# yixuan/ADMM

Measured on AMD Instinct MI355X. Metric: ADMM iterations/sec, Lasso tall n=100000 p=10000 (100-lambda warm-started path), higher is better.
Workload: dtype f32; 1 GPU; admm_lasso tall path (BASELINE configs[1]); n=100000, p=10000, nlambda=100, standardize=True, intercept=True, parallelism=single GPU, step=one cold-started warm-chained lambda path

## Files before the change

admm_amd/csrc/lasso_tall.hip:

```cpp
#include "prep.h"
#include "gemv_kernels.h"
#include "symv_kernels.h"
#include "solvers.h"
#include "sgl_host.h"
#include "box_host.h"
#include "comm.h"
#include "loop_driver.h"
#include "plan_host.h"
#include "peer_device.h"
#include "probe.h"

namespace admm {

struct TallCtl {
    double rho, lam, eps_primal, eps_dual, adj_a, adj_c, tau;
    double a_next, tau_next;
    int mode;
    int restart;
    int iter;
    int lam_idx;
    int done;
    int first;
    int total;
    int fin_idx;
    int fin_niter;
    int pad;
};

struct TallParams {
    int p, nwg, nseg, maxit, nlam, enet;
    long long part_stride;
    double eps_abs, eps_rel, alpha, sqrt_p;
    const double* lambdas;
    const float* XY;
    const float* a_part; const float* b_part;
    const float* dot0; const float* dot1; const float* axp0; const float* axp1;
    long long ldo; int nrb, p32; SymvSched sched;
    float* x; float* z0; float* z1; float* y0; float* y1; float* adj_z; float* adj_y; float* u; float* w;
    TallCtl* ctl;
    double* P;
    float* beta;
    int* niter;
    int* done_host;
#ifdef ADMM_HIP_PROBE
    long long* probe;
#endif
    double* trace;
    long long trace_cap;
    const float* refine_ab;
    long long refine_ld;
    float* state;
    long long state_cap;
    unsigned long long* verdict;
    unsigned long long* early;
    unsigned long long run_tag;
};

__host__ __device__ inline unsigned long long tall_verdict_word(unsigned long long run_tag, int total, bool discard) {
    return run_tag | ((unsigned long long)(unsigned)total << 1) | (discard ? 1ull : 0ull);
}
constexpr int kVerdictShift = 33;
constexpr int kVerdictWords = kSyVerdictReplicas * kSyVerdictStride;

constexpr int kTailThreads = 256;
constexpr int kGateCols = 3;
__host__ __device__ inline const double* tall_norm_rows(const double* P, int nwg, int par) { return P + (size_t)par * nwg * 8; }
__host__ __device__ inline size_t tall_norm_compact(int nwg, int par) { return (size_t)2 * nwg * 8 + (size_t)par * kGateCols * nwg; }
constexpr int kTailLanes = kSySumLanes;
constexpr int kTailElems = kTailThreads / kTailLanes;

__device__ __forceinline__ double tall_load_partial(const double* p, bool in_launch) {
    if (!in_launch) return *p;
    return __longlong_as_double((long long)__hip_atomic_load(reinterpret_cast<const unsigned long long*>(p), __ATOMIC_RELAXED, __HIP_MEMORY_SCOPE_AGENT));
}
__device__ __forceinline__ void tall_store_wt(float* p, float v) {
    __hip_atomic_store(reinterpret_cast<unsigned int*>(p), __float_as_uint(v), __ATOMIC_RELAXED, __HIP_MEMORY_SCOPE_AGENT);
}
__device__ __forceinline__ void tall_store_wt(double* p, double v) {
    __hip_atomic_store(reinterpret_cast<unsigned long long*>(p), (unsigned long long)__double_as_longlong(v), __ATOMIC_RELAXED, __HIP_MEMORY_SCOPE_AGENT);
}

enum { TALL_COLD = 0, TALL_CONVERGED = 1, TALL_ACCELERATE = 2, TALL_RESTART = 3 };
struct TallOutcome {
    int code;
    int fin;
    int done;
    double rp, rd, c;
    __device__ __forceinline__ bool discard() const { return code == TALL_CONVERGED || done != 0; }
    __device__ __forceinline__ int pick() const { return code == TALL_RESTART ? 1 : 0; }
};

template <int NK> struct TallNormReq { double v[2][NK]; };
template <int NK, bool IN_LAUNCH>
__device__ __forceinline__ TallNormReq<NK> tall_norms_request(const double* Pin, int nwg, int rs, int cs) {
    TallNormReq<NK> r;
#pragma unroll
    for (int j = 0; j < 2; ++j) {
        const int w = min((int)threadIdx.x + j * kTailThreads, nwg - 1);
#pragma unroll
        for (int k = 0; k < NK; ++k) r.v[j][k] = tall_load_partial(Pin + (size_t)w * rs + (size_t)k * cs, IN_LAUNCH);
    }
    return r;
}
template <int NK, bool IN_LAUNCH>
__device__ __forceinline__ void tall_norms_sum(const TallNormReq<NK>& r, const double* Pin, int nwg, int rs, int cs, double (&acc)[NK], double* scratch) {
#pragma unroll
    for (int k = 0; k < NK; ++k) acc[k] = 0;
#pragma unroll
    for (int j = 0; j < 2; ++j) {
        const bool live = (int)threadIdx.x + j * kTailThreads < nwg;
#pragma unroll
        for (int k = 0; k < NK; ++k) acc[k] += live ? r.v[j][k] : 0.0;
    }
    for (int w = threadIdx.x + 2 * kTailThreads; w < nwg; w += kTailThreads) {
#pragma unroll
        for (int k = 0; k < NK; ++k) acc[k] += tall_load_partial(Pin + (size_t)w * rs + (size_t)k * cs, IN_LAUNCH);
// ... 4 lines not shown
__device__ __forceinline__ TallOutcome tall_outcome(const TallCtl& in, double r2, double dz2, double daz2, int maxit, int nlam) {
#pragma clang fp contract(off)
    TallOutcome o;
    o.code = TALL_COLD; o.fin = 0; o.done = 0; o.rp = 0; o.rd = 0; o.c = 0;
    if (in.first) return o;
    const double rp = sqrt(r2);
    const double rd = in.rho * sqrt(dz2);
    o.rp = rp; o.rd = rd;
    if (rp < in.eps_primal && rd < in.eps_dual) {
        o.code = TALL_CONVERGED; o.fin = 1;
    } else {
        const double c = fma(in.rho * rp, rp, in.rho * daz2);
        o.c = c;
        o.code = c < 0.999 * in.adj_c ? TALL_ACCELERATE : TALL_RESTART;
        if (in.iter + 1 >= maxit) o.fin = 1;
    }
    if (o.fin && in.lam_idx + 1 >= nlam) o.done = 1;
    return o;
}

struct TallGate {
    const TallCtl* ctl;
    const double* Pin;
    int nwg, maxit, nlam;
    struct Req { TallCtl in; TallNormReq<kGateCols> n; };
    __device__ __forceinline__ void pin() const { asm volatile("" :: "s"(ctl), "s"(Pin), "s"(nwg), "s"(maxit), "s"(nlam)); }
    __device__ __forceinline__ Req request() const {
        Req r;
        r.in = *ctl;
        r.n = tall_norms_request<kGateCols, false>(Pin, nwg, 1, nwg);
        return r;
    }
    __device__ __forceinline__ void sums(const Req& r, double* lds, double (&acc)[kGateCols]) const {
        tall_norms_sum<kGateCols, false>(r.n, Pin, nwg, 1, nwg, acc, lds);
    }
    __device__ __forceinline__ int decide(const Req& r, double* lds) const {
        if (r.in.done) return kSyGateLeave;
        double acc[kGateCols];
        sums(r, lds, acc);
        const TallOutcome o = tall_outcome(r.in, acc[0], acc[1], acc[2], maxit, nlam);
        return o.discard() ? kSyGateLeave : o.pick();
    }
};
static_assert(kSyThreads == kTailThreads, "the tiles and the deciding workgroup share the decision rule: one thread <-> partial mapping");
static_assert(kSyGateScratch >= 6 * (kTailThreads / 64), "block_sum's scratch");

template <bool IN_LAUNCH = false>
__device__ void tall_decide(const TallParams& q, int par) {
    __shared__ double dscratch[6 * (kTailThreads / 64)];
    WIDE_PROBE_DECL
    WIDE_PROBE(0);
    const TallCtl in = q.ctl[par];
    TallCtl* outp = &q.ctl[par ^ 1];
    if (in.done) {
        if (threadIdx.x == 0) { TallCtl o = in; o.fin_idx = -1; *outp = o; }
        return;
    }
    WIDE_PROBE(1);
    double acc[6];
    const double* Pin = tall_norm_rows(q.P, q.nwg, par);
    tall_norms_sum<6, IN_LAUNCH>(tall_norms_request<6, IN_LAUNCH>(Pin, q.nwg, 8, 1), Pin, q.nwg, 8, 1, acc, dscratch);
    if (threadIdx.x != 0) return;
    WIDE_PROBE(2);
    const double x2 = acc[3], z2 = acc[4], y2 = acc[5];
    const TallOutcome oc = tall_outcome(in, acc[0], acc[1], acc[2], q.maxit, q.nlam);
    const double tr_rp = oc.rp, tr_rd = oc.rd, tr_c = oc.c;
    double tr_code = ADMM_TRACE_COLD;
    TallCtl out = in;
    out.first = 0;
    out.fin_idx = -1; out.fin_niter = 0;
    if (oc.code == TALL_COLD) {
        out.mode = 1; out.tau = 0.0; out.restart = 0;
    } else {
        if (oc.code == TALL_CONVERGED) {
            out.fin_idx = in.lam_idx; out.fin_niter = in.iter + 1;
            out.mode = 0;
            tr_code = ADMM_TRACE_CONVERGED;
        } else {
            const double old_c = in.adj_c;
            if (oc.code == TALL_ACCELERATE) {
                out.adj_a = in.a_next; out.adj_c = oc.c; out.tau = in.tau_next; out.restart = 0;
                tr_code = ADMM_TRACE_ACCELERATE;
            } else {
                out.adj_a = 1.0; out.adj_c = old_c / 0.999; out.tau = -1.0; out.restart = 1;
                tr_code = ADMM_TRACE_RESTART;
            }
            out.mode = 1;
            out.iter = in.iter + 1;
            if (oc.fin) {
                out.fin_idx = in.lam_idx; out.fin_niter = q.maxit + 1;
            }
        }
        if (out.fin_idx >= 0) {
            out.lam_idx = in.lam_idx + 1;
            out.iter = 0;
            if (oc.done) out.done = 1;
            else out.lam = q.lambdas[out.lam_idx];
            q.niter[out.fin_idx] = out.fin_niter;
        }
    }
    if (q.verdict != nullptr && oc.discard()) {
        const unsigned long long word = tall_verdict_word(q.run_tag, in.total + 1, true);
        for (int r = 0; r < kSyVerdictReplicas; ++r)
            __hip_atomic_store(q.verdict + (size_t)r * kSyVerdictStride, word, __ATOMIC_RELAXED, __HIP_MEMORY_SCOPE_AGENT);
    }
    out.eps_primal = fmax(sqrt(x2), sqrt(z2)) * q.eps_rel + q.sqrt_p * q.eps_abs;
// ... 573 lines not shown
    ADMM_HIP_CHECK(hipGetLastError());
    read_back(sums_out, ds.get(), 6 * sizeof(double), st.s);
}

struct TallPlan final : LassoPlan {
    DeviceData<float> d;
    LassoProblem pb;
    hipStream_t st;
    admm_stats setup_stats{};
    int p = 0, nlam = 0, nwg = 0;
    long long ldp = 0;
    double rho = 0;
    std::vector<double> lam_user, lam_int;
    GemvTPlan pl;
    SymvPlan sy;
    bool use_sym = false;
    bool shard = false;
    bool peer_fused = false;
    bool peer_one = false;
    int exchange_code = 0;
    CommInfo ci;
    DevBuf<float> ab;
    double dist_flops = 0;
    long long ldv = 0;
    DevBuf<float> XY, M, a_part, b_part, x, z0, z1, y0, y1, adj_z, adj_y, u, w, beta;
    DevBuf<int> niter;
    DevBuf<double> P, dlam;
    DevBuf<TallCtl> ctl;
    DevBuf<unsigned long long> verdict;
    bool verdict_on = false, verdict_mid = false;
    bool decide_first = false;
    SymvPacked pk;
    bool packed = false;
    unsigned long long run_no = 0;
    TallParams q{};
    bool refine = false;
    DevBuf<float> Mg, rab, ruw;
    DevBuf<double> dD0, dD1, xD0, xD1;
    bool grouped = false, sgl = false;
    DevBuf<int2> gtiles;
    DevBuf<GroupCoord> gcoord;
    DevBuf<double> gl1;
    GroupTailParams gq{};
    int mt = 0;
    int mt_rhs = 2;
    DevBuf<float> uw, mdot, maxp;
    DevBuf<double> roww;
    MtTailParams mq{};
    bool box = false;
    DevBuf<double> bpf;
    DevBuf<float> blo, bhi;
    BoxTailParams bq{};
    BoxClamp clamp;
    PinnedFlag hflag;
#ifdef ADMM_HIP_PROBE
    DevBuf<long long> probe;
#endif
    float* hbeta = nullptr;

    std::vector<hipEvent_t> ev_pool;

    ~TallPlan() override {
        if (hbeta) (void)hipHostFree(hbeta);
        for (auto e : ev_pool) (void)hipEventDestroy(e);
    }

    TallPlan(DeviceData<float>&& data, const LassoProblem& prob, hipStream_t stream) : d(std::move(data)), pb(prob), st(stream) {
        const int n = d.n;
        p = d.p;
        admm_stats& S = setup_stats;
        S.branch = 0;
        S.t_h2d = d.t_h2d; S.t_standardize = d.t_std;
        ldp = round_up(p, 128);

        shard = pb.dist;
        ci = shard ? comm_info() : CommInfo();
        const long long nt = d.n_total > 0 ? d.n_total : n;
        if (d.xy.get()) {
            ADMM_REQUIRE(!shard && d.gram.get() && d.ldgram == ldp, "Gram-form data needs X'X next to X'y");
            XY = std::move(d.xy);
        } else if (pb.penalty == Penalty::MULTITASK) {
            mt = pb.nresp;
            ADMM_REQUIRE(mt >= 1 && mt <= kMtMax && d.nresp == mt && d.Ymt.get() && (int)pb.row_weight.size() == p, "internal: multi-task sizes");
            XY.alloc((size_t)mt * ldp); XY.zero(st);
            for (int k = 0; k < mt; ++k) gemv_t_simple<float>(d.X.get(), d.ldx, n, p, d.Ymt.get() + (size_t)k * d.ldx, XY.get() + (size_t)k * ldp, st);
        } else {
            XY.alloc(ldp); XY.zero(st);
            gemv_t_simple<float>(d.X.get(), d.ldx, n, p, d.Y.get(), XY.get(), st);
            if (shard) allreduce_sum_f32(XY.get(), (size_t)p, st);
        }
        sgl = pb.penalty == Penalty::SGL; grouped = sgl || pb.penalty == Penalty::GROUP; box = pb.penalty == Penalty::BOX;
        ADMM_REQUIRE(pb.penalty == Penalty::PLAIN || (!shard && !opt_on(Opt::REFINE) && (box || !pb.enet) && (mt > 0) == (pb.penalty == Penalty::MULTITASK)),
                     "internal: a penalty other than the Lasso's is the plain single-device tall solver on column data");
        ADMM_REQUIRE(!grouped || ((int)pb.group_start.size() == (int)pb.group_weight.size() + 1 && pb.group_start.back() == p), "internal: group sizes");
        ADMM_REQUIRE((int)pb.l1_weight.size() == (sgl ? p : 0), "internal: l1 weights belong to the sparse-group lasso");
        ADMM_REQUIRE(!box || ((int)pb.box_lower.size() == p && (int)pb.box_upper.size() == p && (int)pb.penalty_factor.size() == p), "internal: box sizes");
        float lambda0 = 0.f;
        switch (pb.penalty) {
        case Penalty::PLAIN: lambda0 = device_absmax<float>(XY.get(), p, st); break;
        case Penalty::GROUP: lambda0 = group_lambda0(); break;
        case Penalty::SGL: lambda0 = sgl_plan_lambda0(); break;
        case Penalty::MULTITASK: lambda0 = mt_lambda0(); break;
        case Penalty::BOX: lambda0 = box_plan_lambda0(); break;
        }
        if (pb.enet) lambda0 = (float)(lambda0 / ((double)(float)pb.alpha + 0.0001));

        nlam = make_path_grid<float>(pb, lambda0, nt, (double)d.scaleY, lam_user, lam_int);

        {
            size_t free_b = 0, total_b = 0;
            ADMM_HIP_CHECK(hipMemGetInfo(&free_b, &total_b));
            free_b += pool_cached_bytes();
            if (opt_set(Opt::TEST_FREE_BYTES)) free_b = (size_t)opt_int(Opt::TEST_FREE_BYTES, 0);
            const bool have_gram = d.gram.get() && d.ldgram == ldp;
            const bool inv64_wanted = p < 4096 || opt_is(Opt::INVERSE, "f64");
            const double mat = (double)ldp * (double)ldp * 4.0;
            const double need = (have_gram ? 0.0 : mat) + (inv64_wanted ? 2.0 * mat : 0.5 * mat) + (opt_on(Opt::REFINE) ? mat : 0.0) +
// ... 139 lines not shown
        if (shard) { q.a_part = ab.get(); q.b_part = ab.get() + ldp; q.nseg = 1; }
        q.dot0 = sy.dot0.get(); q.dot1 = sy.dot1.get(); q.axp0 = sy.axp0.get(); q.axp1 = sy.axp1.get();
        q.ldo = sy.ldo; q.nrb = sy.nrb; q.p32 = sy.p32; q.sched = sy.sched;
        q.refine_ab = refine ? rab.get() : nullptr; q.refine_ld = ldv;
        q.x = x.get(); q.z0 = z0.get(); q.z1 = z1.get(); q.y0 = y0.get(); q.y1 = y1.get();
        q.adj_z = adj_z.get(); q.adj_y = adj_y.get(); q.u = u.get(); q.w = w.get();
        q.ctl = ctl.get(); q.P = P.get(); q.beta = beta.get(); q.niter = niter.get();
        q.done_host = hflag.p;
        const int level = (int)opt_int(Opt::SYMV_VERDICT, 3);
        verdict_on = use_sym && !shard && !refine && !mt && level != 0;
        decide_first = verdict_on && level == 3;
        verdict_mid = level == 2;
        if (verdict_on) {
            verdict.alloc(kVerdictWords + kSyEarlySlots * kSyVerdictStride); verdict.zero(st);
            q.verdict = decide_first ? nullptr : verdict.get();
            q.early = verdict.get() + kVerdictWords;
        }
        packed = false;
        t_pack_info[0] = t_pack_info[1] = t_pack_info[2] = t_pack_info[3] = 0;
        if (decide_first && opt_int(Opt::SYMV_PACK, 1) != 0) {
            size_t free_b = 0, total_b = 0;
            ADMM_HIP_CHECK(hipMemGetInfo(&free_b, &total_b));
            free_b += pool_cached_bytes();
            if (opt_set(Opt::TEST_FREE_BYTES)) free_b = (size_t)opt_int(Opt::TEST_FREE_BYTES, 0);
            if ((double)SymvPacked::bytes_for(sy) <= 0.97 * (double)free_b) {
                packed = pk.build(sy, M.get(), ldp, st, (int)opt_int(Opt::SYMV_PACK_ESC, kSpEscCap));
                t_pack_info[1] = (long long)pk.escapes; t_pack_info[2] = (long long)pk.overflowed; t_pack_info[3] = (long long)pk.bytes();
                if (!packed) pk.release();
            }
            t_pack_info[0] = packed ? 1 : 0;
        }
#ifdef ADMM_HIP_PROBE
        probe.alloc((size_t)4096 * 4 * 8); probe.zero(st);
        q.probe = probe.get();
        sy.probe = probe.get();
#endif

        if (mt) {
            static const int kAutoRhs[kMtMax] = {2, 4, 8, 8, 12, 12, 8, 8, 4, 4, 12, 12, 4, 4, 8, 8};
            mt_rhs = kAutoRhs[mt - 1];
            if (const OptValue* v = opt(Opt::MT_RHS)) { if (v->i > 0) mt_rhs = kSyNR[v->i - 1]; }
            uw.alloc((size_t)2 * mt * ldv); uw.zero(st);
            const size_t ds = (size_t)sy.nrb * sy.ldo, as = (size_t)sy.nax_rows * sy.ldo;
            mdot.alloc((size_t)2 * mt * ds); maxp.alloc((size_t)2 * mt * as);
            mdot.zero(st); maxp.zero(st);
            x.zero(st); z0.zero(st); z1.zero(st); y0.zero(st); y1.zero(st); adj_z.zero(st); adj_y.zero(st);
            roww.alloc(p);
            ADMM_HIP_CHECK(hipMemcpyAsync(roww.get(), pb.row_weight.data(), (size_t)p * sizeof(double), hipMemcpyHostToDevice, st));
            mq.m = mt; mq.ldv = ldv; mq.ldxy = ldp; mq.uw = uw.get();
            mq.dot = mdot.get(); mq.axp = maxp.get(); mq.dot_stride = (long long)ds; mq.axp_stride = (long long)as;
            mq.row_w = roww.get();
        }
        ADMM_HIP_CHECK(hipHostMalloc(reinterpret_cast<void**>(&hbeta), (size_t)nlam * p * npl * sizeof(float), hipHostMallocDefault));
        comm_stream_sync(st);
    }

    float box_plan_lambda0() {
        std::vector<float> lo(p), hi(p), h(p);
        for (int j = 0; j < p; ++j) {
            lo[j] = box_round_lower(box_to_std(pb.box_lower[j], (double)d.scaleX[j], (double)d.scaleY));
            hi[j] = box_round_upper(box_to_std(pb.box_upper[j], (double)d.scaleX[j], (double)d.scaleY));
        }
        clamp.set(pb.box_lower, pb.box_upper);
        bpf.alloc((size_t)p); blo.alloc((size_t)p); bhi.alloc((size_t)p);
        ADMM_HIP_CHECK(hipMemcpyAsync(bpf.get(), pb.penalty_factor.data(), (size_t)p * sizeof(double), hipMemcpyHostToDevice, st));
        ADMM_HIP_CHECK(hipMemcpyAsync(blo.get(), lo.data(), (size_t)p * sizeof(float), hipMemcpyHostToDevice, st));
        ADMM_HIP_CHECK(hipMemcpyAsync(bhi.get(), hi.data(), (size_t)p * sizeof(float), hipMemcpyHostToDevice, st));
        read_back(h.data(), XY.get(), (size_t)p * sizeof(float), st);
        bq.pf = bpf.get(); bq.lo = blo.get(); bq.hi = bhi.get();
        return box_lambda0(h.data(), p, lo.data(), hi.data(), pb.penalty_factor.data());
    }

    float mt_lambda0() {
        std::vector<float> h((size_t)mt * ldp);
        read_back(h.data(), XY.get(), h.size() * sizeof(float), st);
        double best = 0.0;
        for (int j = 0; j < p; ++j) {
            if (!(pb.row_weight[j] > 0)) continue;
            double s2 = 0.0;
            for (int k = 0; k < mt; ++k) { const double v = (double)h[(size_t)k * ldp + j]; s2 += v * v; }
            best = std::max(best, std::sqrt(s2) / pb.row_weight[j]);
        }
        return (float)best;
    }
    double mt_partial_floats() const {
        const double nrb = (double)((p + kSyRB - 1) / kSyRB), ldo = nrb * kSyRB;
        return 2.0 * mt * (nrb + (double)((p + 31) / 32)) * ldo;
    }

    float group_lambda0() {
        std::vector<float> h(p);
        read_back(h.data(), XY.get(), (size_t)p * sizeof(float), st);
        double best = 0.0;
        for (size_t g = 0; g + 1 < pb.group_start.size(); ++g) {
            if (!(pb.group_weight[g] > 0)) continue;
            double s2 = 0.0;
            for (int j = pb.group_start[g]; j < pb.group_start[g + 1]; ++j) s2 += (double)h[j] * (double)h[j];
            best = std::max(best, std::sqrt(s2) / pb.group_weight[g]);
        }
        return (float)best;
    }

    float sgl_plan_lambda0() {
        std::vector<float> h(p);
        read_back(h.data(), XY.get(), (size_t)p * sizeof(float), st);
        return sgl_lambda0(h.data(), pb.group_start, pb.l1_weight, pb.group_weight);
// ... 14 lines not shown
            ADMM_REQUIRE(gn >= 1 && gn <= kGroupMax && gs == first + count, "internal: bad group partition");
            for (int j = gs; j < gs + gn; ++j)
                coord[j] = GroupCoord{gs, gn, sgl && gn == 1 ? sgl_single_weight(pb.l1_weight[j], wg) : wg};
            if (count + gn > kTailElems) flush();
            count += gn;
            if (gn > kTailElems) flush();
        }
        flush();
        gtiles.alloc(tiles.size()); gcoord.alloc(coord.size());
        ADMM_HIP_CHECK(hipMemcpyAsync(gtiles.get(), tiles.data(), tiles.size() * sizeof(int2), hipMemcpyHostToDevice, st));
        ADMM_HIP_CHECK(hipMemcpyAsync(gcoord.get(), coord.data(), coord.size() * sizeof(GroupCoord), hipMemcpyHostToDevice, st));
        if (sgl) {
            gl1.alloc((size_t)p);
            ADMM_HIP_CHECK(hipMemcpyAsync(gl1.get(), pb.l1_weight.data(), (size_t)p * sizeof(double), hipMemcpyHostToDevice, st));
        }
        comm_stream_sync(st);
        gq.tiles = gtiles.get(); gq.coord = gcoord.get(); gq.l1 = sgl ? gl1.get() : nullptr;
        return (int)tiles.size();
    }

    Records records() override { return {st, 5ll * p * std::max(mt, 1), &q.trace, &q.trace_cap, &q.state, &q.state_cap}; }

    void read_system(float* out, long long ld) override {
        if (!refine) throw Error(ADMM_ERR_INVALID_ARG, "the system matrix is only kept with ADMM_HIP_REFINE=1");
        ADMM_REQUIRE(out != nullptr && ld >= p, "bad output for the system matrix");
        ADMM_HIP_CHECK(hipMemcpy2D(out, (size_t)ld * sizeof(float), Mg.get(), (size_t)ldp * sizeof(float), (size_t)p * sizeof(float), (size_t)p, hipMemcpyDeviceToHost));
    }

    void run(LassoResult& res) override {
        admm_stats S = setup_stats;
        S.xupdate_variant = shard ? 2 : (use_sym ? 1 : 0);
        S.exchange_variant = exchange_code;
        S.refine = refine ? 1 : 0;
        S.factor_flops = dist_flops;
        res.lambda = lam_user;
        beta.zero(st); niter.zero(st);
        q.run_tag = ++run_no << kVerdictShift;
        const int init_n = std::max(p, 2 * nwg * (8 + kGateCols));
        for (int k = 0; k < std::max(mt, 1); ++k) {
            TallParams qk = q;
            if (mt) {
                const size_t o = (size_t)k * ldv;
                qk.x += o; qk.z0 += o; qk.z1 += o; qk.y0 += o; qk.y1 += o; qk.adj_z += o; qk.adj_y += o;
                qk.XY += (size_t)k * ldp; qk.u = uw.get() + (size_t)(2 * k) * ldv; qk.w = uw.get() + (size_t)(2 * k + 1) * ldv;
            }
            hipLaunchKernelGGL(tall_init_kernel, dim3((init_n + 255) / 256), dim3(256), 0, st, qk, rho, lam_int[0]);
        }
        if (q.state != nullptr && mt)
            ADMM_HIP_CHECK(hipMemcpy2DAsync(q.state, (size_t)p * sizeof(float), XY.get(), (size_t)ldp * sizeof(float), (size_t)p * sizeof(float),
                                            (size_t)mt, hipMemcpyDeviceToDevice, st));
        else if (q.state != nullptr)
            ADMM_HIP_CHECK(hipMemcpyAsync(q.state, XY.get(), (size_t)p * sizeof(float), hipMemcpyDeviceToDevice, st));
        *hflag.p = 0;
#ifdef ADMM_HIP_PROBE
        sy.probe_idx = 0;
#endif

        const int batch = batch_iters(pb.batch_iters, 32);
        const int stride = pb.profile_stride;
        size_t nev = 0;
        const auto done_at = [&](long long g) -> const int* { return &ctl.get()[(int)(g & 1)].done; };
        const LoopTimes lt = run_until_done(st, done_at, batch, (long long)nlam * ((long long)pb.opts.maxit + 2) + 4, [&](long long g) {
            const int par = (int)(g & 1);
            const bool sample = stride > 0 && (g % stride) == stride / 2 && nev < 8192;
            hipEvent_t e0 = nullptr, e1 = nullptr;
            if (sample) {
                while (ev_pool.size() < nev + 2) {
                    hipEvent_t e; ADMM_HIP_CHECK(hipEventCreate(&e));
                    ev_pool.push_back(e);
                }
                e0 = ev_pool[nev]; e1 = ev_pool[nev + 1];
                nev += 2;
            }
            const TallDecideExtra dec{q, par};
            SymvVerdict vd;
            if (verdict_on && !decide_first) { vd.words = verdict.get(); vd.discard = tall_verdict_word(q.run_tag, (int)(g + 1), true); vd.early = verdict.get() + kVerdictWords; vd.mid = verdict_mid; }
            const int* skip = &ctl.get()[par].done;
            const auto xupdate = [&] {
                if (decide_first) {
                    const TallGate gate{ctl.get() + par, P.get() + tall_norm_compact(nwg, par), nwg, q.maxit, q.nlam};
                    if (packed) symv_launch_one_packed(sy, pk, u.get(), w.get(), skip, st, gate, q.early, dec, e0, e1);
                    else sy.launch_one(M.get(), ldp, u.get(), w.get(), skip, st, gate, q.early, dec, e0, e1);
                }
                else if (use_sym) sy.launch(M.get(), ldp, u.get(), w.get(), skip, st, dec, e0, e1, vd);
                else launch_gemv_t<float, 2, 4, TallDecideExtra>(pl, M.get(), ldp, p, p, u.get(), w.get(), a_part.get(), b_part.get(), ldp, skip, st, dec, e0, e1);
            };
            const auto group_tail = [&] {
                void (*tail)(TallParams, int, GroupTailParams) =
                    decide_first ? (sgl ? tall_group_tail_kernel<TAIL_SYMV1, true> : tall_group_tail_kernel<TAIL_SYMV1>)
                    : use_sym ? (sgl ? tall_group_tail_kernel<TAIL_SYMV, true> : tall_group_tail_kernel<TAIL_SYMV>)
                            : (sgl ? tall_group_tail_kernel<TAIL_GEMV, true> : tall_group_tail_kernel<TAIL_GEMV>);
                hipLaunchKernelGGL(tail, dim3(nwg), dim3(kTailThreads), 0, st, q, par, gq);
            };
            if (mt) {
                const int nvec = 2 * mt;
                for (int r0 = 0; r0 < nvec; r0 += mt_rhs) {
                    SymvNArgs a;
                    a.A = M.get(); a.lda = ldp; a.p = p;
                    a.v = uw.get() + (size_t)r0 * ldv; a.vstride = ldv;
                    a.dot = mdot.get() + (size_t)r0 * mq.dot_stride; a.dot_stride = mq.dot_stride;
                    a.axp = maxp.get() + (size_t)r0 * mq.axp_stride; a.axp_stride = mq.axp_stride;
                    a.nvec = std::min(mt_rhs, nvec - r0); a.ldo = sy.ldo; a.tiles = sy.tiles.get(); a.skip = skip;
                    hipEvent_t es = r0 == 0 ? e0 : nullptr, ee = r0 + mt_rhs >= nvec ? e1 : nullptr;
                    if (r0 == 0) symvn_launch(sy, mt_rhs, a, st, dec, es, ee);
                    else symvn_launch(sy, mt_rhs, a, st, SymvNoExtra(), es, ee);
                }
                hipLaunchKernelGGL(tall_mt_tail_kernel, dim3(nwg), dim3(kTailThreads), 0, st, q, par, mq);
            } else if (grouped) {
                xupdate();
                group_tail();
            } else if (shard && peer_fused) {
                sy.launch(M.get(), ldp, u.get(), w.get(), skip, st, dec, e0, e1);
                const PeerExchange ex = comm_peer_begin((size_t)2 * ldp * sizeof(float));
                if (peer_one) {
                    hipLaunchKernelGGL(tall_tail_kernel<TAIL_PEER1>, dim3(nwg), dim3(kTailThreads), 0, st, q, par, ex);
                } else {
                    hipLaunchKernelGGL(tall_shard_push_kernel, dim3(nwg), dim3(kTailThreads), 0, st, q, ex, ldp, skip);
                    hipLaunchKernelGGL(tall_tail_kernel<TAIL_PEER>, dim3(nwg), dim3(kTailThreads), 0, st, q, par, ex);
                }
            } else if (shard) {
                sy.launch(M.get(), ldp, u.get(), w.get(), skip, st, dec, e0, e1);
                hipLaunchKernelGGL(tall_shard_reduce_kernel, dim3(nwg), dim3(kTailThreads), 0, st, q, ab.get(), ldp, skip);
                allreduce_sum_f32(ab.get(), (size_t)2 * ldp, st);
                hipLaunchKernelGGL(tall_tail_kernel<TAIL_GEMV>, dim3(nwg), dim3(kTailThreads), 0, st, q, par, PeerExchange{});
            } else if (use_sym && refine) {
                sy.launch(M.get(), ldp, u.get(), w.get(), skip, st, dec, e0, e1);
                hipLaunchKernelGGL(tall_shard_reduce_kernel, dim3(nwg), dim3(kTailThreads), 0, st, q, rab.get(), ldv, skip);
                SymvArgsD ad;
                ad.A = Mg.get(); ad.lda = ldp; ad.p = p; ad.v0 = rab.get(); ad.v1 = rab.get() + ldv;
                ad.dot0 = dD0.get(); ad.dot1 = dD1.get(); ad.axp0 = xD0.get(); ad.axp1 = xD1.get(); ad.ldo = sy.ldo; ad.tiles = sy.tiles.get(); ad.skip = skip;
                hipLaunchKernelGGL(symv2_lower_f64acc_kernel, dim3(sy.ntiles), dim3(kSyThreads), 0, st, ad);
                hipLaunchKernelGGL(tall_refine_resid_kernel, dim3(nwg), dim3(kTailThreads), 0, st, q, dD0.get(), dD1.get(), xD0.get(), xD1.get(),
                                   ruw.get(), ruw.get() + ldv, skip);
                sy.launch(M.get(), ldp, ruw.get(), ruw.get() + ldv, skip, st, SymvNoExtra());
                hipLaunchKernelGGL(tall_tail_kernel<TAIL_SYMV>, dim3(nwg), dim3(kTailThreads), 0, st, q, par, PeerExchange{});
            } else if (box) {
                xupdate();
                if (decide_first) hipLaunchKernelGGL(tall_box_tail_kernel<TAIL_SYMV1>, dim3(nwg), dim3(kTailThreads), 0, st, q, par, bq);
                else if (use_sym) hipLaunchKernelGGL(tall_box_tail_kernel<TAIL_SYMV>, dim3(nwg), dim3(kTailThreads), 0, st, q, par, bq);
                else hipLaunchKernelGGL(tall_box_tail_kernel<TAIL_GEMV>, dim3(nwg), dim3(kTailThreads), 0, st, q, par, bq);
            } else {
                xupdate();
                if (decide_first) hipLaunchKernelGGL(tall_tail_kernel<TAIL_SYMV1>, dim3(nwg), dim3(kTailThreads), 0, st, q, par, PeerExchange{});
                else if (use_sym) hipLaunchKernelGGL(tall_tail_kernel<TAIL_SYMV>, dim3(nwg), dim3(kTailThreads), 0, st, q, par, PeerExchange{});
                else hipLaunchKernelGGL(tall_tail_kernel<TAIL_GEMV>, dim3(nwg), dim3(kTailThreads), 0, st, q, par, PeerExchange{});
            }
        }, LoopOpts{shard ? nullptr : hflag.p, 0, false});
        S.t_loop = lt.wall_s; S.loop_ms_events = lt.events_ms; S.xupdate_launches = lt.launched;
        const CtlPair<TallCtl> hctl = read_ctl(ctl.get());
        unsigned long long early = 0;
        if (verdict_on) {
            std::vector<unsigned long long> slots((size_t)kSyEarlySlots * kSyVerdictStride);
            ADMM_HIP_CHECK(hipMemcpy(slots.data(), verdict.get() + kVerdictWords, slots.size() * sizeof(unsigned long long), hipMemcpyDeviceToHost));
            for (int k = 0; k < kSyEarlySlots; ++k) early += slots[(size_t)k * kSyVerdictStride];
        }
        t_early_exits = (long long)early;
        WIDE_PROBE_DUMP(probe);
        if (nev > 0) {
            double tot = 0;
            for (size_t k = 0; k + 1 < nev; k += 2) {
                float m1 = 0.f;
                ADMM_HIP_CHECK(hipEventElapsedTime(&m1, ev_pool[k], ev_pool[k + 1]));
                tot += m1;
            }
            S.xupdate_samples = (long long)(nev / 2);
            S.xupdate_ms_avg = tot / (double)(nev / 2);
        }

        ADMM_HIP_CHECK(hipMemcpyAsync(hbeta, beta.get(), (size_t)nlam * p * std::max(mt, 1) * sizeof(float), hipMemcpyDeviceToHost, st));
        comm_stream_sync(st);
        if (mt) {
            const size_t col = (size_t)p + 1;
            std::vector<float> bk;
            res.beta.assign(col * mt * nlam, 0.f);
            for (int k = 0; k < mt; ++k) {
                S.total_iter = read_out_path<float>(d, hbeta + (size_t)k * p, nlam, niter.get(), col, 0, res.niter, bk, INT_MAX, (size_t)mt * p, &d.meanYs[k]);
                for (int l = 0; l < nlam; ++l) std::memcpy(res.beta.data() + ((size_t)l * mt + k) * col, bk.data() + (size_t)l * col, col * sizeof(float));
            }
        } else {
            S.total_iter = read_out_path<float>(d, hbeta, nlam, niter.get(), (size_t)p + 1, 0, res.niter, res.beta, INT_MAX, 0, nullptr, &clamp);
        }
        decisions = hctl.c[0].done ? hctl.total() : 0;
        res.stats = S;
    }
};

std::unique_ptr<LassoPlan> make_tall_plan(DeviceData<float>&& d, const LassoProblem& pb, hipStream_t st) {
    return std::unique_ptr<LassoPlan>(new TallPlan(std::move(d), pb, st));
}

}
```

admm_amd/csrc/loop_driver.h:

```cpp
#pragma once
#include "admm_internal.h"
#include "comm.h"

namespace admm {

struct LoopTimes {
    double wall_s = 0;
    double events_ms = 0;
    long long launched = 0;
};

struct PinnedFlag {
    int* p = nullptr;
    PinnedFlag() { ADMM_HIP_CHECK(hipHostMalloc(reinterpret_cast<void**>(&p), sizeof(int), hipHostMallocDefault)); *p = 0; }
    ~PinnedFlag() { if (p) pinned_free(p); }
    PinnedFlag(const PinnedFlag&) = delete;
    PinnedFlag& operator=(const PinnedFlag&) = delete;
};

struct LoopOpts {
    const volatile int* h_flag = nullptr;
    long long g_start = 0;
    bool grow = true;
};

inline const int* poll_word(const int* w, long long) { return w; }
template <typename P> auto poll_word(P& at, long long g) -> decltype(at(g)) { return at(g); }

template <typename P, typename F>
inline LoopTimes run_until_done(hipStream_t st, P d_done, int batch, long long max_iters, F&& enqueue, const LoopOpts& o = LoopOpts()) {
    const TraceRange trace_range("admm:loop");
    const volatile int* h_flag = o.h_flag;
    const long long g_start = o.g_start;
    int* h_done = nullptr;
    if (h_flag == nullptr) {
        ADMM_HIP_CHECK(hipHostMalloc(reinterpret_cast<void**>(&h_done), 2 * sizeof(int), hipHostMallocDefault));
        h_done[0] = h_done[1] = 0;
    }
    struct HostFree { void* p; ~HostFree() { if (p) pinned_free(p); } } hf{h_done};
    const CommLockstep lockstep;
    const int batch0 = batch;
    int npoll = 0;
    Event ev0, ev1, poll[2];
    LoopTimes t;
    comm_stream_sync(st);
    const double t0 = now_s();
    ADMM_HIP_CHECK(hipEventRecord(ev0.e, st));
    long long g = g_start;
    auto enqueue_batch = [&](int slot) {
        for (int k = 0; k < batch; ++k, ++g) enqueue(g);
        if (h_flag == nullptr) ADMM_HIP_CHECK(hipMemcpyAsync(&h_done[slot], poll_word(d_done, g), sizeof(int), hipMemcpyDeviceToHost, st));
        ADMM_HIP_CHECK(hipEventRecord(poll[slot].e, st));
    };
    int slot = 0;
    enqueue_batch(slot);
    ADMM_HIP_CHECK(hipGetLastError());
    bool done = false;
    while (!done) {
        enqueue_batch(slot ^ 1);
        comm_event_sync(poll[slot].e);
        comm_check();
        done = h_flag ? (*h_flag != 0) : (h_done[slot] != 0);
        slot ^= 1;
        if (o.grow && h_flag && (++npoll & 3) == 0 && batch < 4 * batch0) batch *= 2;
        if (!done && g - g_start > max_iters + 2 * batch)
            throw Error(ADMM_ERR_INTERNAL, "ADMM loop: iteration bound exceeded without completion");
    }
    ADMM_HIP_CHECK(hipEventRecord(ev1.e, st));
    comm_stream_sync(st);
    t.wall_s = now_s() - t0;
    float ms = 0.f;
    ADMM_HIP_CHECK(hipEventElapsedTime(&ms, ev0.e, ev1.e));
    t.events_ms = ms;
    t.launched = g - g_start;
    return t;
}

}
```

admm_amd/csrc/options.h:

```cpp
#pragma once
#include <limits>
#include <string>
#include <vector>

namespace admm {

enum class OptKind { Flag, Int, Real, Choice, Text, Sched, Devices };
struct OptAccepts {
    OptKind kind;
    double lo = 0, hi = 0;
    const char* choices = nullptr;
};
constexpr OptAccepts Flag() { return {OptKind::Flag, 0, 1}; }
constexpr OptAccepts Int(double lo, double hi) { return {OptKind::Int, lo, hi}; }
constexpr OptAccepts Real(double lo, double hi) { return {OptKind::Real, lo, hi}; }
constexpr OptAccepts Choice(const char* c) { return {OptKind::Choice, 0, 0, c}; }
constexpr OptAccepts Text() { return {OptKind::Text}; }
constexpr OptAccepts Sched() { return {OptKind::Sched}; }
constexpr OptAccepts Devices() { return {OptKind::Devices}; }
constexpr double kPositive = std::numeric_limits<double>::min();

#define ADMM_OPTIONS(X)                                                                                                                  \
    X(BATCH_ITERS, Int(1, 1 << 20), "iterations enqueued between two host polls (rounded up to even; default per solver)")             \
    X(PROFILE_STRIDE, Int(0, 1 << 30), "time every k-th tall x-update launch with HIP events (0: off)")                                 \
    X(GRAM, Choice("rocblas|oneshot"), "tall Gram through rocBLAS / host input transferred before the Gram is built")                    \
    X(GRAM_SPLIT, Choice("0|f16x2|bf16x3"), "tall Gram of order >= ~4000: exact fp32 kernel / fp16 x 2 (default) / bf16 x 3")          \
    X(GRAM_B3_KTILES, Int(0, 1 << 20), "K tiles per launch of the 16-bit split Gram (0: one launch)")                                   \
    X(FACTOR, Choice("rocsolver"), "Cholesky + inverse through rocSOLVER / rocBLAS instead of the hand-written kernels")                \
    X(INVERSE, Choice("f32|f64"), "precision the cached inverse is built in")                                                           \
    X(XUPDATE, Choice("sym|gemv|full"), "tall x-update: symmetric lower-triangle kernel / full-matrix mat-vec (gemv and full alike)")   \
    X(SYMV_SCHED, Sched(), "tall x-update: column-segment widths of the long / short row strips and the split between them")           \
    X(SYMV_VERDICT, Choice("0|1|2|3"), "tall x-update: discarded launches stream on / leave on block 0's word at start / also mid-tile / every tile decides first, one vector (default)") \
    X(SYMV_PACK, Choice("0|1"), "tall x-update, decide-first form: stream the fp32 inverse / its exact 29-bit copy (default)")          \
    X(SYMV_PACK_ESC, Int(0, 4096), "tall x-update: entries a tile of the 29-bit copy may hold outside its exponent window (default 32; one tile beyond it: the fp32 stream)") \
    X(REFINE, Flag(), "tall path: refine every x-update with a double-precision residual")                                               \
    X(DIST_FACTOR, Flag(), "row-sharded tall solver: 0 = every rank factorises the whole all-reduced Gram")                            \
    X(CV_DOWNDATE, Flag(), "cross-validation folds' Grams as down-dates of the full-data Gram: 1 always, 0 never")                      \
    X(PREP_FUSED, Flag(), "0: convert, column statistics and standardisation as separate sweeps over X")                                \
    X(H2D, Choice("pageable"), "host inputs through plain hipMemcpy instead of the pinned staging ring")                                 \
    X(POOL_MB, Int(0, 1 << 30), "cache of released device blocks, megabytes (0: off)")                                                  \
    X(WIDE_FUSE, Flag(), "wide path: 0 = three launches per iteration")                                                                  \
    X(WIDE_TGLOBAL, Flag(), "wide path: 1 = t through global memory instead of LDS")                                                     \
    X(WIDE_SPRAD, Choice("gram"), "wide path: spectral radius from the explicit n x n Gram")                                            \
    X(WIDE_SCREEN, Choice("0|8|16|auto"), "wide path: screen the regular steps never / 8-bit code / fp16 copy / chosen at any size")    \
    X(WIDE_SCREEN_STATS, Flag(), "wide path: print the screen's counts")                                                                 \
    X(WIDE_PERSIST, Flag(), "wide path: 0 = no persistent active-set stretches")                                                         \
    X(WIDE_PERSIST_COLS, Flag(), "column-sharded wide solver: 0 = no persistent active-set stretches")                                  \
    X(WIDE_ROWS_C, Int(1, 32), "wide path: column groups of the 2-D stretch (kept only when it fits with the problem's row groups)")    \
    X(WIDE_PERSIST_STATS, Flag(), "wide path: print the stretch statistics")                                                             \
    X(PAR_ONEPASS, Flag(), "consensus solver: 0 = the reference's two products per Woodbury worker")                                    \
    X(PAR_ONEPASS_TAU, Real(0, 1e300), "one-pass Woodbury workers: threshold of the cancellation guard (0: never fall back)")           \
    X(PAR_ONEPASS_STATS, Flag(), "one-pass Woodbury workers: print how many worker-iterations took the dense pass")                     \
    X(PAR_FUSE_PZ, Flag(), "consensus solver: 0 = pack and z as two launches")                                                           \
    X(PAR_BATCH, Flag(), "consensus solver: 0 = one launch per worker and product")                                                      \
    X(PAR_DEVICES, Devices(), "admm_hip_parlasso / admm_hip_parbp over several devices in one process")                                \
    X(TEST_PAR_FAIL_RANK, Int(0, 63), "test hook: this rank of an in-process call fails before its first exchange")                    \
    X(PEER_FUSED, Choice("0|1|2"), "PEER back-end: 0 = the generic all-reduce, 2 = producer and consumer as two launches")             \
    X(PEER_MEM, Choice("uncached"), "PEER exchange buffers as uncached device memory")                                                   \
    X(COMM_SLOT_BYTES, Int(4096, 1ll << 40), "payload capacity of one PEER / SHM exchange (rounded down to 16 bytes)")                 \
    X(COMM_TIMEOUT_S, Real(kPositive, 1e300), "wait bound of the per-iteration exchanges, seconds")                                    \
    X(COMM_PATIENT_TIMEOUT_S, Real(kPositive, 1e300), "wait bound of setup reductions and replica joins, seconds")                     \
    X(LAD_HAT, Flag(), "LAD: 0 = the general projection also for n <= 2000")                                                            \
    X(LAD_ONEPASS, Flag(), "LAD: 0 = the reference's two products per iteration")                                                      \
    X(QUANT_SLOTS, Int(0, 8), "admm_hip_quantreg, admm_hip_huber: fits per pass over X on the one-pass branch: 0 = automatic, 1 = serial, else at most that many") \
    X(MT_RHS, Choice("0|2|4|8|12"), "admm_hip_mtlasso: right-hand sides per pass over the cached inverse (0: automatic)")               \
    X(BP_ONEPASS, Flag(), "basis pursuit: 0 = the reference's two products per iteration")                                             \
    X(SBP_GRAM, Flag(), "admm_hip_parbp: 0 = the direct launches on every active-set iteration")                                       \
    X(SBP_GRAM_CAP, Int(1, 1024), "admm_hip_parbp: most columns of the Gram-space matrix (rounded to multiples of 8)")                 \
    X(SBP_GRAM_CARRY, Flag(), "admm_hip_parbp: 0 = every Gram-space stretch starts from the direct launches' n-vectors")              \
    X(SBP_SCREEN, Flag(), "admm_hip_parbp: screen the regular iterations always / never")                                             \
    X(SBP_SCREEN_STATS, Flag(), "admm_hip_parbp: print the screen's counts")                                                           \
    X(SBP_WGS, Int(1, 1 << 20), "admm_hip_parbp: workgroups of the x-update launches")                                                 \
    X(SBP_SHARE, Int(1, 1 << 20), "admm_hip_parbp: smallest share of a block's non-zero list a workgroup takes")                      \
    X(SBP_TEST_DELAY_US, Int(0, 1000000), "test hook: every even workgroup of a Gram-space launch starts that many us late")           \
    X(TEST_RESIDENT_WGS, Int(0, 1ll << 40), "test hook: pretend the device holds that many resident workgroups")                      \
    X(TEST_FREE_BYTES, Int(0, 1ll << 52), "test hook: pretend the device has that many bytes free")                                    \
    X(PROBE_OUT, Text(), "dev build with in-kernel timestamps (-DADMM_HIP_PROBE): file the probe records go to")

enum class Opt : int {
#define ADMM_OPT_ID(id, accepts, summary) id,
    ADMM_OPTIONS(ADMM_OPT_ID)
#undef ADMM_OPT_ID
};
constexpr int kNumOptions = 0
#define ADMM_OPT_COUNT(id, accepts, summary) +1
    ADMM_OPTIONS(ADMM_OPT_COUNT)
#undef ADMM_OPT_COUNT
// ... 33 lines not shown
```

admm_amd/csrc/plan_host.h:

```cpp
#pragma once
#include "solvers.h"
#include "comm.h"
#include "box_host.h"
#include <climits>

namespace admm {

template <typename Round, typename Stored>
int make_path_grid(const LassoProblem& pb, double lambda0, long long n, double scaleY, std::vector<double>& user, std::vector<Stored>& internal) {
    user = make_lambda_grid(pb, lambda0, (int)n, scaleY);
    internal.resize(user.size());
    for (size_t i = 0; i < user.size(); ++i) internal[i] = (Stored)(Round)(user[i] * (double)n / scaleY);
    return (int)user.size();
}

template <typename T>
long long read_out_path(const DeviceData<T>& d, const T* snap, int nlam, const int* dev_niter, size_t stride, long long col_offset,
                        std::vector<int>& niter, std::vector<T>& beta, int niter_clip = INT_MAX, size_t snap_stride = 0,
                        const T* mean_y = nullptr, const BoxClamp* box = nullptr) {
    if (snap_stride == 0) snap_stride = (size_t)d.p;
    niter.assign(nlam, 0);
    ADMM_HIP_CHECK(hipMemcpy(niter.data(), dev_niter, (size_t)nlam * sizeof(int), hipMemcpyDeviceToHost));
    beta.assign(stride * nlam, T(0));
    long long tot = 0;
    for (int l = 0; l < nlam; ++l) {
        T b0 = 0;
        T* out = beta.data() + (size_t)l * stride + 1 + col_offset;
        recover_coef<T>(d, mean_y ? *mean_y : d.meanY, snap + (size_t)l * snap_stride, &b0, out);
        if (box != nullptr && box->on() && box->apply(out, d.p) && (d.flag & 2)) {
            T acc = T(0);
            for (int j = 0; j < d.p; ++j) acc += out[j] * d.meanX[j];
            b0 = (mean_y ? *mean_y : d.meanY) - acc;
        }
        beta[(size_t)l * stride] = b0;
        tot += std::min(niter[l], niter_clip);
    }
    return tot;
}

template <typename Ctl>
struct CtlPair {
    Ctl c[2];
    long long total() const { return std::max(c[0].total, c[1].total); }
    const Ctl& finished() const { return c[0].done ? c[0] : c[1]; }
};
template <typename Ctl>
CtlPair<Ctl> read_ctl(const Ctl* dev) {
    CtlPair<Ctl> h;
    ADMM_HIP_CHECK(hipMemcpy(h.c, dev, sizeof(h.c), hipMemcpyDeviceToHost));
    return h;
}

inline int exchange_variant(bool sharded, bool fused, bool one) { return !sharded ? 0 : (!fused ? 1 : (one ? 3 : 2)); }

struct ExchangeForm { bool fused = false, one = false; int variant = 0; };
inline ExchangeForm peer_exchange_form(bool sharded, const CommInfo& ci, const void* one_kernel, int block, long long grid) {
    ExchangeForm f;
    f.fused = sharded && ci.backend == COMM_PEER && !opt_is(Opt::PEER_FUSED, "0");
    if (f.fused) {
        int occ = 0;
        ADMM_HIP_CHECK(hipOccupancyMaxActiveBlocksPerMultiprocessor(&occ, one_kernel, block, 0));
        f.one = grid * 2 <= resident_workgroups(occ) && !opt_is(Opt::PEER_FUSED, "2");
    }
    f.variant = exchange_variant(sharded, f.fused, f.one);
    return f;
}

}
```

Baseline: 29020 iterations/s.

## Overlap per-lambda coefficient readout and recovery with the running ADMM loop

The decide kernel now writes the index of the last finished lambda into a second pinned host word. While the host polls the loop, a callback copies the newly finished betas and iteration counts on a separate stream and recovers coefficients on the host. After the loop only the remaining lambdas are copied, so host-side recovery is meant to hide behind GPU work. The risks are extra copy traffic on a second stream during the loop and host work added to each poll, which could delay launching the next batch.

```diff
diff --git a/admm_amd/csrc/lasso_tall.hip b/admm_amd/csrc/lasso_tall.hip
--- a/admm_amd/csrc/lasso_tall.hip
+++ b/admm_amd/csrc/lasso_tall.hip
@@ -62,6 +62,7 @@
 constexpr int kVerdictShift = 33;
 constexpr int kVerdictWords = kSyVerdictReplicas * kSyVerdictStride;
 
+constexpr int kTallProgress = 1;
 constexpr int kTailThreads = 256;
 constexpr int kGateCols = 3;
 __host__ __device__ inline const double* tall_norm_rows(const double* P, int nwg, int par) { return P + (size_t)par * nwg * 8; }
@@ -172,6 +173,7 @@
     WIDE_PROBE(0);
     const TallCtl in = q.ctl[par];
     TallCtl* outp = &q.ctl[par ^ 1];
+    if (in.fin_idx >= 0 && threadIdx.x == 0) q.done_host[kTallProgress] = in.fin_idx + 1;
     if (in.done) {
         if (threadIdx.x == 0) { TallCtl o = in; o.fin_idx = -1; *outp = o; }
         return;
@@ -851,7 +853,7 @@
     DevBuf<float> blo, bhi;
     BoxTailParams bq{};
     BoxClamp clamp;
-    PinnedFlag hflag;
+    PinnedFlag hflag{2};
 #ifdef ADMM_HIP_PROBE
     DevBuf<long long> probe;
 #endif
@@ -859,9 +861,73 @@
 
     std::vector<hipEvent_t> ev_pool;
 
+    struct Small {
+        TallCtl ctl[2];
+        unsigned long long slots[kSyEarlySlots * kSyVerdictStride];
+    };
+    Small* hsmall = nullptr;
+    int* hniter = nullptr;
+    std::unique_ptr<Stream> ro_stream;
+    std::vector<hipEvent_t> ro_ev;
+    struct ReadOut {
+        TallPlan* plan; LassoResult* res;
+        bool sized = false;
+        int copied = 0;
+        int recovered = 0;
+        size_t nrange = 0, nready = 0;
+        std::vector<int> end;
+        long long total_iter = 0;
+    };
+    void readout_size(ReadOut& r) {
+        if (r.sized) return;
+        r.res->beta.assign(((size_t)p + 1) * nlam, 0.f);
+        r.res->niter.assign(nlam, 0);
+        r.sized = true;
+    }
+    void readout_enqueue(ReadOut& r, int upto, hipStream_t s) {
+        if (upto <= r.copied) return;
+        const size_t l0 = (size_t)r.copied, cnt = (size_t)(upto - r.copied);
+        ADMM_HIP_CHECK(hipMemcpyAsync(hbeta + l0 * p, beta.get() + l0 * p, cnt * p * sizeof(float), hipMemcpyDeviceToHost, s));
+        ADMM_HIP_CHECK(hipMemcpyAsync(hniter + l0, niter.get() + l0, cnt * sizeof(int), hipMemcpyDeviceToHost, s));
+        while (ro_ev.size() <= r.nrange) {
+            hipEvent_t e; ADMM_HIP_CHECK(hipEventCreateWithFlags(&e, hipEventDisableTiming));
+            ro_ev.push_back(e);
+        }
+        ADMM_HIP_CHECK(hipEventRecord(ro_ev[r.nrange], s));
+        r.end.push_back(upto);
+        ++r.nrange;
+        r.copied = upto;
+    }
+    void readout_drain(ReadOut& r, bool wait) {
+        for (; r.nready < r.nrange; ++r.nready) {
+            if (wait) ADMM_HIP_CHECK(hipEventSynchronize(ro_ev[r.nready]));
+            else {
+                const hipError_t q = hipEventQuery(ro_ev[r.nready]);
+                if (q == hipErrorNotReady) { (void)hipGetLastError(); return; }
+                ADMM_HIP_CHECK(q);
+            }
+            const int l1 = r.end[r.nready];
+            r.total_iter += read_out_range<float>(d, hbeta, r.recovered, l1, (size_t)p + 1, 0, hniter, r.res->beta.data(), INT_MAX, 0, nullptr, &clamp);
+            for (int l = r.recovered; l < l1; ++l) r.res->niter[l] = hniter[l];
+            r.recovered = l1;
+        }
+    }
+    static void readout_poll(void* arg) {
+        ReadOut& r = *static_cast<ReadOut*>(arg);
+        TallPlan& t = *r.plan;
+        t.readout_size(r);
+        const int seen = *static_cast<const volatile int*>(t.hflag.p + kTallProgress);
+        const int c = std::min(seen, t.nlam);
+        t.readout_enqueue(r, c, t.ro_stream->s);
+        t.readout_drain(r, false);
+    }
+
     ~TallPlan() override {
         if (hbeta) (void)hipHostFree(hbeta);
+        if (hsmall) (void)hipHostFree(hsmall);
+        if (hniter) (void)hipHostFree(hniter);
         for (auto e : ev_pool) (void)hipEventDestroy(e);
+        for (auto e : ro_ev) (void)hipEventDestroy(e);
     }
 
     TallPlan(DeviceData<float>&& data, const LassoProblem& prob, hipStream_t stream) : d(std::move(data)), pb(prob), st(stream) {
@@ -1107,6 +1173,8 @@
             mq.row_w = roww.get();
         }
         ADMM_HIP_CHECK(hipHostMalloc(reinterpret_cast<void**>(&hbeta), (size_t)nlam * p * npl * sizeof(float), hipHostMallocDefault));
+        ADMM_HIP_CHECK(hipHostMalloc(reinterpret_cast<void**>(&hsmall), sizeof(Small), hipHostMallocDefault));
+        ADMM_HIP_CHECK(hipHostMalloc(reinterpret_cast<void**>(&hniter), (size_t)nlam * sizeof(int), hipHostMallocDefault));
         comm_stream_sync(st);
     }
 
@@ -1227,6 +1295,15 @@
         else if (q.state != nullptr)
             ADMM_HIP_CHECK(hipMemcpyAsync(q.state, XY.get(), (size_t)p * sizeof(float), hipMemcpyDeviceToDevice, st));
         *hflag.p = 0;
+        hflag.p[kTallProgress] = 0;
+        const bool overlap = !shard && mt == 0 && !opt_off(Opt::READOUT_OVERLAP);
+        ReadOut ro{this, &res};
+        LoopOpts lopts{shard ? nullptr : hflag.p, 0, false};
+        if (overlap) {
+            if (!ro_stream) ro_stream.reset(new Stream());
+            lopts.on_poll = &TallPlan::readout_poll;
+            lopts.on_poll_arg = &ro;
+        }
 #ifdef ADMM_HIP_PROBE
         sy.probe_idx = 0;
 #endif
@@ -1320,16 +1397,24 @@
                 else if (use_sym) hipLaunchKernelGGL(tall_tail_kernel<TAIL_SYMV>, dim3(nwg), dim3(kTailThreads), 0, st, q, par, PeerExchange{});
                 else hipLaunchKernelGGL(tall_tail_kernel<TAIL_GEMV>, dim3(nwg), dim3(kTailThreads), 0, st, q, par, PeerExchange{});
             }
-        }, LoopOpts{shard ? nullptr : hflag.p, 0, false});
+        }, lopts);
         S.t_loop = lt.wall_s; S.loop_ms_events = lt.events_ms; S.xupdate_launches = lt.launched;
-        const CtlPair<TallCtl> hctl = read_ctl(ctl.get());
+        CtlPair<TallCtl> hctl;
         unsigned long long early = 0;
-        if (verdict_on) {
-            std::vector<unsigned long long> slots((size_t)kSyEarlySlots * kSyVerdictStride);
-            ADMM_HIP_CHECK(hipMemcpy(slots.data(), verdict.get() + kVerdictWords, slots.size() * sizeof(unsigned long long), hipMemcpyDeviceToHost));
-            for (int k = 0; k < kSyEarlySlots; ++k) early += slots[(size_t)k * kSyVerdictStride];
-        }
-        t_early_exits = (long long)early;
+        if (overlap) {
+            ADMM_HIP_CHECK(hipMemcpyAsync(hsmall->ctl, ctl.get(), sizeof(hsmall->ctl), hipMemcpyDeviceToHost, st));
+            if (verdict_on) ADMM_HIP_CHECK(hipMemcpyAsync(hsmall->slots, verdict.get() + kVerdictWords, sizeof(hsmall->slots), hipMemcpyDeviceToHost, st));
+            readout_size(ro);
+            readout_enqueue(ro, nlam, st);
+            readout_drain(ro, false);
+        } else {
+            hctl = read_ctl(ctl.get());
+            if (verdict_on) {
+                std::vector<unsigned long long> slots((size_t)kSyEarlySlots * kSyVerdictStride);
+                ADMM_HIP_CHECK(hipMemcpy(slots.data(), verdict.get() + kVerdictWords, slots.size() * sizeof(unsigned long long), hipMemcpyDeviceToHost));
+                for (int k = 0; k < kSyEarlySlots; ++k) early += slots[(size_t)k * kSyVerdictStride];
+            }
+        }
         WIDE_PROBE_DUMP(probe);
         if (nev > 0) {
             double tot = 0;
@@ -1342,6 +1427,18 @@
             S.xupdate_ms_avg = tot / (double)(nev / 2);
         }
 
+        if (overlap) {
+            comm_stream_sync(st);
+            readout_drain(ro, true);
+            hctl.c[0] = hsmall->ctl[0]; hctl.c[1] = hsmall->ctl[1];
+            if (verdict_on) for (int k = 0; k < kSyEarlySlots; ++k) early += hsmall->slots[(size_t)k * kSyVerdictStride];
+            t_early_exits = (long long)early;
+            S.total_iter = ro.total_iter;
+            decisions = hctl.c[0].done ? hctl.total() : 0;
+            res.stats = S;
+            return;
+        }
+        t_early_exits = (long long)early;
         ADMM_HIP_CHECK(hipMemcpyAsync(hbeta, beta.get(), (size_t)nlam * p * std::max(mt, 1) * sizeof(float), hipMemcpyDeviceToHost, st));
         comm_stream_sync(st);
         if (mt) {
diff --git a/admm_amd/csrc/loop_driver.h b/admm_amd/csrc/loop_driver.h
--- a/admm_amd/csrc/loop_driver.h
+++ b/admm_amd/csrc/loop_driver.h
@@ -12,7 +12,10 @@
 
 struct PinnedFlag {
     int* p = nullptr;
-    PinnedFlag() { ADMM_HIP_CHECK(hipHostMalloc(reinterpret_cast<void**>(&p), sizeof(int), hipHostMallocDefault)); *p = 0; }
+    explicit PinnedFlag(int words = 1) {
+        ADMM_HIP_CHECK(hipHostMalloc(reinterpret_cast<void**>(&p), (size_t)words * sizeof(int), hipHostMallocDefault));
+        for (int k = 0; k < words; ++k) p[k] = 0;
+    }
     ~PinnedFlag() { if (p) pinned_free(p); }
     PinnedFlag(const PinnedFlag&) = delete;
     PinnedFlag& operator=(const PinnedFlag&) = delete;
@@ -22,6 +25,8 @@
     const volatile int* h_flag = nullptr;
     long long g_start = 0;
     bool grow = true;
+    void (*on_poll)(void*) = nullptr;
+    void* on_poll_arg = nullptr;
 };
 
 inline const int* poll_word(const int* w, long long) { return w; }
@@ -60,6 +65,7 @@
         enqueue_batch(slot ^ 1);
         comm_event_sync(poll[slot].e);
         comm_check();
+        if (o.on_poll != nullptr) o.on_poll(o.on_poll_arg);
         done = h_flag ? (*h_flag != 0) : (h_done[slot] != 0);
         slot ^= 1;
         if (o.grow && h_flag && (++npoll & 3) == 0 && batch < 4 * batch0) batch *= 2;
diff --git a/admm_amd/csrc/options.h b/admm_amd/csrc/options.h
--- a/admm_amd/csrc/options.h
+++ b/admm_amd/csrc/options.h
@@ -33,6 +33,7 @@
     X(SYMV_VERDICT, Choice("0|1|2|3"), "tall x-update: discarded launches stream on / leave on block 0's word at start / also mid-tile / every tile decides first, one vector (default)") \
     X(SYMV_PACK, Choice("0|1"), "tall x-update, decide-first form: stream the fp32 inverse / its exact 29-bit copy (default)")          \
     X(SYMV_PACK_ESC, Int(0, 4096), "tall x-update: entries a tile of the 29-bit copy may hold outside its exponent window (default 32; one tile beyond it: the fp32 stream)") \
+    X(READOUT_OVERLAP, Flag(), "tall path, one rank: 0 = every lambda is copied and recovered on the host after the loop, none while it runs") \
     X(REFINE, Flag(), "tall path: refine every x-update with a double-precision residual")                                               \
     X(DIST_FACTOR, Flag(), "row-sharded tall solver: 0 = every rank factorises the whole all-reduced Gram")                            \
     X(CV_DOWNDATE, Flag(), "cross-validation folds' Grams as down-dates of the full-data Gram: 1 always, 0 never")                      \
diff --git a/admm_amd/csrc/plan_host.h b/admm_amd/csrc/plan_host.h
--- a/admm_amd/csrc/plan_host.h
+++ b/admm_amd/csrc/plan_host.h
@@ -15,17 +15,13 @@
 }
 
 template <typename T>
-long long read_out_path(const DeviceData<T>& d, const T* snap, int nlam, const int* dev_niter, size_t stride, long long col_offset,
-                        std::vector<int>& niter, std::vector<T>& beta, int niter_clip = INT_MAX, size_t snap_stride = 0,
-                        const T* mean_y = nullptr, const BoxClamp* box = nullptr) {
+long long read_out_range(const DeviceData<T>& d, const T* snap, int l0, int l1, size_t stride, long long col_offset, const int* niter,
+                         T* beta, int niter_clip = INT_MAX, size_t snap_stride = 0, const T* mean_y = nullptr, const BoxClamp* box = nullptr) {
     if (snap_stride == 0) snap_stride = (size_t)d.p;
-    niter.assign(nlam, 0);
-    ADMM_HIP_CHECK(hipMemcpy(niter.data(), dev_niter, (size_t)nlam * sizeof(int), hipMemcpyDeviceToHost));
-    beta.assign(stride * nlam, T(0));
     long long tot = 0;
-    for (int l = 0; l < nlam; ++l) {
+    for (int l = l0; l < l1; ++l) {
         T b0 = 0;
-        T* out = beta.data() + (size_t)l * stride + 1 + col_offset;
+        T* out = beta + (size_t)l * stride + 1 + col_offset;
         recover_coef<T>(d, mean_y ? *mean_y : d.meanY, snap + (size_t)l * snap_stride, &b0, out);
         if (box != nullptr && box->on() && box->apply(out, d.p) && (d.flag & 2)) {
             T acc = T(0);
@@ -36,6 +32,16 @@
         tot += std::min(niter[l], niter_clip);
     }
     return tot;
+}
+
+template <typename T>
+long long read_out_path(const DeviceData<T>& d, const T* snap, int nlam, const int* dev_niter, size_t stride, long long col_offset,
+                        std::vector<int>& niter, std::vector<T>& beta, int niter_clip = INT_MAX, size_t snap_stride = 0,
+                        const T* mean_y = nullptr, const BoxClamp* box = nullptr) {
+    niter.assign(nlam, 0);
+    ADMM_HIP_CHECK(hipMemcpy(niter.data(), dev_niter, (size_t)nlam * sizeof(int), hipMemcpyDeviceToHost));
+    beta.assign(stride * nlam, T(0));
+    return read_out_range<T>(d, snap, 0, nlam, stride, col_offset, niter.data(), beta.data(), niter_clip, snap_stride, mean_y, box);
 }
 
 template <typename Ctl>
```

Result: no change. 29200 iterations/s (median of 6 runs) (+0.6%).
